# dkales/dpf-go

Measured on AMD Instinct MI355X. Metric: DPF leaf points/sec (EvalFull logN=20, batched keys) + AES blocks/sec, higher is better.
Workload: dtype u32

## Files before the change

### dpf-go_amd/csrc/dpf_capi.hip

```cpp
#include <hip/hip_runtime.h>
#include <sched.h>
#include <stdint.h>
#include <stdio.h>
#include <stdlib.h>
#include <string.h>
#include <sys/mman.h>

#include <algorithm>
#include <atomic>
#include <condition_variable>
#include <functional>
#include <memory>
#include <mutex>
#include <unordered_map>
#include <string>
#include <thread>
#include <vector>

#include "../../include/dpf_hip.h"
#include "dpf_internal.hpp"
#include "bs_kernels.hpp"
#include "dpf_kernels.hpp"
#include "pir_kernels.hpp"
#include "pir_update_plan.hpp"
// ... 313 lines not shown
    void* frontier;
};

TreeWs tree_ws(void* work, size_t nk, uint32_t stop) {
    uint8_t* p = static_cast<uint8_t*>(work);
    TreeWs w;
    w.ek = reinterpret_cast<uint32_t*>(p);
    p += align256(nk * dpfk::ek_words(stop) * 4);
    w.ekb = reinterpret_cast<uint32_t*>(p);
    p += align256(nk * dpfk::bs_key_words(stop) * 4);
    w.frontier = p;
    return w;
}

bool want_bs() { return g_aes_impl.load(std::memory_order_relaxed) == DPF_AES_BITSLICED; }

hipError_t expand_keys(const uint8_t* d_keys, size_t klen, size_t nk, uint32_t stop, const TreeWs& w, hipStream_t st,
                       bool bs) {
    if (bs) return dpfk::launch_unpack_both(d_keys, klen, nk, stop, w.ek, w.ekb, st);
    return dpfk::launch_unpack(d_keys, klen, nk, stop, w.ek, st);
}

hipError_t run_tree(const TreeWs& w, size_t k0, size_t n, uint32_t stop, uint32_t prefix_bits, uint64_t prefix,
                    uint8_t* out, uint64_t stride, hipStream_t st, bool bs) {
    if (bs && dpfk::bs_applicable(stop, prefix_bits))
        return dpfk::launch_evalfull_bs(w.ek + k0 * dpfk::ek_words(stop), w.ekb + k0 * dpfk::bs_key_words(stop), n, stop,
                                        prefix_bits, prefix, out, stride, w.frontier, st);
    return dpfk::launch_evalfull(w.ek + k0 * dpfk::ek_words(stop), n, stop, prefix_bits, prefix, out, stride, st);
}

hipError_t tree_from_keys(const uint8_t* d_keys, size_t klen, size_t nk, uint32_t stop, uint32_t prefix_bits,
                          uint64_t prefix, uint8_t* out, uint64_t stride, void* d_work, hipStream_t st, bool bs,
                          bool* expanded) {
    if (!bs && dpfk::evalfull_raw_ok(nk, stop, prefix_bits)) {
        *expanded = false;
        return dpfk::launch_evalfull_raw(d_keys, klen, nk, stop, prefix_bits, prefix, out, stride, st);
    }
    *expanded = true;
    const TreeWs w = tree_ws(d_work, nk, stop);
    hipError_t e = expand_keys(d_keys, klen, nk, stop, w, st, bs);
    return e != hipSuccess ? e : run_tree(w, 0, nk, stop, prefix_bits, prefix, out, stride, st, bs);
}

constexpr size_t kStageBytes = (size_t)32 << 20;
constexpr size_t kSlabMinOut = (size_t)8 << 20;

int ensure_staging(Dev& d, size_t chunk_cap) {
    if (!d.cst) {
        HIP_TRY(hipStreamCreateWithFlags(&d.cst, hipStreamNonBlocking));
        for (int i = 0; i < 2; ++i) {
            HIP_TRY(hipEventCreateWithFlags(&d.ev_k[i], hipEventDisableTiming));
            HIP_TRY(hipEventCreateWithFlags(&d.ev_c[i], hipEventDisableTiming));
        }
    }
    HIP_TRY(hipError_t(d.out.ensure(2 * chunk_cap)));
    for (int i = 0; i < 2; ++i) HIP_TRY(d.pin[i].ensure(chunk_cap));
    return DPF_OK;
}

bool prefault_output() {
    static const bool on = [] {
        const char* e = getenv("DPF_PREFAULT_OUTPUT");
        return e && e[0] == '1';
    }();
    return on;
}

void hint_hugepages(uint8_t* p, size_t n) {
    if (n < ((size_t)64 << 20) || !prefault_output()) return;
    const uintptr_t a = ((uintptr_t)p + ((1u << 21) - 1)) & ~(uintptr_t)((1u << 21) - 1);
    const uintptr_t e = ((uintptr_t)p + n) & ~(uintptr_t)((1u << 21) - 1);
    if (e > a) (void)madvise((void*)a, e - a, MADV_HUGEPAGE);
// ... 391 lines not shown
        if (!raw) HIP_TRY(expand_keys(dk, klen, 1, stop, w, d.st, bs));
        return pipeline_d2h(d, (size_t)1 << extra, sub, [&](size_t j, uint8_t* dbuf, size_t& bytes, size_t& off) {
            const uint64_t p = ((uint64_t)lo << extra) + j;
            if (raw) HIP_TRY(dpfk::launch_evalfull_raw(dk, klen, 1, stop, pb + extra, p, dbuf, sub, d.st));
            else HIP_TRY(run_tree(w, 0, 1, stop, pb + extra, p, dbuf, sub, d.st, bs));
            bytes = sub;
            off = lo * slab + j * sub;
            return DPF_OK;
        }, out + lo * slab, slab, lo * slab);
    });
}

int dpf_evalfull_subtree_dev(int device, const uint8_t* d_keys, size_t klen, size_t nkeys, uint32_t logN,
                             uint32_t prefix_bits, uint64_t prefix, uint8_t* d_out, void* d_work, void* stream) {
    if (int rc = check_key(klen, logN)) return rc;
    const uint32_t stop = stop_of(logN);
    if (prefix_bits > stop || (prefix_bits < 64 && (prefix >> prefix_bits) != 0))
        return fail(DPF_ERR_PARAM, "dpf: subtree prefix out of range");
    if (nkeys == 0) return DPF_OK;
    DeviceGuard g(device);
    CuScope cus(stream);
    const bool bs = want_bs();
    bool expanded = false;
    forget_expanded(d_work);
    HIP_TRY(tree_from_keys(d_keys, klen, nkeys, stop, prefix_bits, prefix, d_out, (uint64_t)16 << (stop - prefix_bits),
                           d_work, (hipStream_t)stream, bs, &expanded));
    if (expanded) note_expanded(d_work, nkeys, stop, bs);
    return DPF_OK;
}

int dpf_evalfull_batch_dev(int device, const uint8_t* d_keys, size_t klen, size_t nkeys, uint32_t logN,
                           uint8_t* d_out, void* d_work, void* stream) {
    return dpf_evalfull_subtree_dev(device, d_keys, klen, nkeys, logN, 0, 0, d_out, d_work, stream);
}

size_t dpf_eval_workspace_size(size_t nkeys, size_t pts_per_key, uint32_t logN) {
    return std::max<size_t>(16, eval_work_bytes(nkeys, pts_per_key, logN));
}

uint32_t dpf_eval_frontier_level(uint32_t logN, size_t pts_per_key) {
    return logN > 63 ? 0 : dpfk::eval_frontier_level(stop_of(logN), pts_per_key);
}

int dpf_eval_batch_dev(int device, const uint8_t* d_keys, size_t klen, size_t nkeys, const uint64_t* d_xs,
                       size_t ppk, uint32_t logN, uint8_t* d_out, void* d_work, size_t work_bytes, void* stream) {
    if (int rc = check_key(klen, logN, false)) return rc;
    if (nkeys == 0 || ppk == 0) return DPF_OK;
    const uint32_t stop = stop_of(logN);
    const size_t ekb = pir_ek_bytes(nkeys, logN);
    if (work_bytes < nkeys * dpfk::ek_words(stop) * 4) return fail(DPF_ERR_PARAM, "dpf: Eval workspace too small");
    if (d_xs == nullptr || d_out == nullptr || d_keys == nullptr || (reinterpret_cast<uintptr_t>(d_xs) & 7u) != 0)
        return fail(DPF_ERR_PARAM, "dpf: d_keys/d_xs/d_out must be device pointers, d_xs 8-byte aligned");
    DeviceGuard g(device);
    CuScope cus(stream);
    forget_expanded(d_work);
    HIP_TRY(dpfk::launch_unpack(d_keys, klen, nkeys, stop, (uint32_t*)d_work, (hipStream_t)stream));
    void* frontier = work_bytes > ekb ? (uint8_t*)d_work + ekb : nullptr;
    HIP_TRY(dpfk::launch_eval((const uint32_t*)d_work, stop, logN, d_xs, nkeys * ppk, ppk, d_out, frontier,
                              work_bytes > ekb ? work_bytes - ekb : 0, (hipStream_t)stream));
    return DPF_OK;
}

int dpf_expand_keys_dev(int device, const uint8_t* d_keys, size_t klen, size_t nkeys, uint32_t logN, void* d_work,
                        void* stream) {
    if (int rc = check_key(klen, logN)) return rc;
    DeviceGuard g(device);
// ... 486 lines not shown
```

### dpf-go_amd/csrc/dpf_kernels.hip

```cpp
#include <hip/hip_runtime.h>
#include <stdint.h>
#include <stdlib.h>

#include <algorithm>
#include <atomic>
#include <cmath>
#include <type_traits>
#include "aes_consts.hpp"
#include "aes_ttable.hpp"
#include "dpf_kernels.hpp"
#include "wave_prio.hpp"
#include "tree_ops.hpp"

namespace dpfk {

#ifdef DPF_WAVE_TIMES
constexpr uint64_t kWaveTimesMax = 1u << 16;
__device__ uint64_t g_wave_times[5 * kWaveTimesMax];
#endif

struct Ctx {
    const uint8_t* tab;
    uint32_t lo;
    KeySrc ks;
// ... 550 lines not shown
    const uint64_t pairs = nblocks / 2;
    if (pairs == 0) return hipSuccess;
    const dim3 grid((uint32_t)((pairs + kBlock - 1) / kBlock));
    if (right)
        hipLaunchKernelGGL(k_mmo_tt<true>, grid, dim3(kBlock), 0, st, reinterpret_cast<const uint4*>(in),
                           reinterpret_cast<uint4*>(out), pairs, reps);
    else
        hipLaunchKernelGGL(k_mmo_tt<false>, grid, dim3(kBlock), 0, st, reinterpret_cast<const uint4*>(in),
                           reinterpret_cast<uint4*>(out), pairs, reps);
    return hipGetLastError();
}

hipError_t launch_unpack(const uint8_t* keys, uint64_t key_len, uint64_t nkeys, uint32_t stop, uint32_t* ek,
                         hipStream_t st) {
    const uint64_t n = nkeys * ((uint64_t)stop + 2);
    if (n == 0) return hipSuccess;
    const uint32_t blocks = (uint32_t)((n + 255) / 256);
    hipLaunchKernelGGL(k_unpack, dim3(blocks), dim3(256), 0, st, keys, key_len, nkeys, stop, ek);
    return hipGetLastError();
}

static thread_local int t_cu_budget = 0;
void set_cu_budget(int cus) { t_cu_budget = cus; }
int cu_budget() { return t_cu_budget; }
int cu_count() {
    if (t_cu_budget > 0) return t_cu_budget;
    int dev = 0, cus = 256;
    if (hipGetDevice(&dev) != hipSuccess ||
        hipDeviceGetAttribute(&cus, hipDeviceAttributeMultiprocessorCount, dev) != hipSuccess)
        cus = 256;
    return cus;
}

static uint32_t pick_block(uint64_t n, uint32_t maxb) {
    const uint64_t cus = (uint64_t)cu_count();
    uint32_t b = 64;
    while (b < maxb && n > cus * b) b <<= 1;
    return b;
}

struct TreeShape {
    uint32_t d, block;
};
static TreeShape pick_shape(uint32_t span, uint64_t nkeys, bool nodes, uint32_t prefix_bits) {
    static const int forced = [] {
        const char* e = getenv("DPF_SUBTREE_DEPTH");
        return e ? atoi(e) : -1;
    }();
    const uint32_t dmax = span < kMaxD ? span : kMaxD;
    auto threads = [&](uint32_t dd) { return span - dd >= 40 ? ~0ull : nkeys << (span - dd); };
    auto block = [&](uint32_t dd) {
        return pick_block(threads(dd), !nodes && dd >= kBigMinD ? (uint32_t)kTreeBlockBig : (uint32_t)kTreeBlock);
    };
    if (forced >= 0) {
        const uint32_t d = dmax < (uint32_t)forced ? dmax : (uint32_t)forced;
        return {d, block(d)};
    }
    constexpr double kLat = 1.9e-6;
    constexpr double kPerWave = 0.2e-6;
    const double wave_slots = 64.0 * cu_count();
    uint32_t best = dmax;
    double best_t = 1e30;
    for (int dd = (int)dmax; dd >= 0; --dd) {
        const uint32_t d = (uint32_t)dd;
        double walk = (double)(span - d), lat = 0.0;
        const double w = (double)threads(d) / wave_slots;
        const double rounds = w > 16.0 ? std::ceil(w / 16.0) : 1.0;
        const double per = w > 16.0 ? 16.0 * kPerWave : std::max(kLat, w * kPerWave);
        const uint32_t W = 31u - (uint32_t)__builtin_clz(block(d));
        if (W >= 7 && span - d >= W) {
            walk = (double)(W - 6);
            lat = (double)(span + prefix_bits - d - W + 6) * kLat;
        }
        const double work = walk + (nodes ? 2.0 : 3.0) * (double)(1u << d) - 2.0;
        const double t = rounds * (lat + work * std::max(kLat, per));
        if (t < best_t * 0.98) {
            best_t = t;
            best = d;
        }
    }
    return {best, block(best)};
}

struct TreeLaunch {
    uint32_t d;
    uint32_t ltop;
    uint32_t units_log;
    uint64_t nunits, sub_base;
    dim3 grid, block;
};
static TreeLaunch tree_launch(uint64_t nkeys, uint32_t depth, uint32_t prefix_bits, uint64_t prefix, bool nodes) {
    const TreeShape sh = pick_shape(depth - prefix_bits, nkeys, nodes, prefix_bits);
    TreeLaunch t;
    t.d = sh.d;
    t.ltop = depth - sh.d;
    t.units_log = t.ltop - prefix_bits;
    t.nunits = nkeys << t.units_log;
    t.sub_base = prefix << t.units_log;
    t.grid = dim3((uint32_t)((t.nunits + sh.block - 1) / sh.block));
    t.block = dim3(sh.block);
    return t;
}
template <class F>
static void with_depth(uint32_t d, F&& f) {
    switch (d) {
        case 0: return f(std::integral_constant<int, 0>{});
        case 1: return f(std::integral_constant<int, 1>{});
        case 2: return f(std::integral_constant<int, 2>{});
        case 3: return f(std::integral_constant<int, 3>{});
        case 4: return f(std::integral_constant<int, 4>{});
        case 5: return f(std::integral_constant<int, 5>{});
        case 6: return f(std::integral_constant<int, 6>{});
        default: return f(std::integral_constant<int, 7>{});
    }
}

template <bool NODES>
static hipError_t launch_tree(const uint32_t* ek, uint64_t nkeys, uint32_t stop, uint32_t depth,
                              uint32_t prefix_bits, uint64_t prefix, uint8_t* out, uint8_t* out_t,
                              uint64_t out_stride, hipStream_t st) {
    const TreeLaunch t = tree_launch(nkeys, depth, prefix_bits, prefix, NODES);
    if (t.nunits == 0) return hipSuccess;
    with_depth(t.d, [&](auto dd) {
        constexpr int D = decltype(dd)::value;
        if (t.units_log >= 6)
            hipLaunchKernelGGL((k_evalfull<D, true, NODES>), t.grid, t.block, 0, st, ek, stop, t.nunits, t.units_log,
                               t.ltop, t.sub_base, out, out_t, out_stride);
        else
            hipLaunchKernelGGL((k_evalfull<D, false, NODES>), t.grid, t.block, 0, st, ek, stop, t.nunits, t.units_log,
                               t.ltop, t.sub_base, out, out_t, out_stride);
    });
    return hipGetLastError();
}

bool evalfull_raw_ok(uint64_t nkeys, uint32_t stop, uint32_t prefix_bits) {
    static const bool on = [] {
        const char* e = getenv("DPF_RAW_KEYS");
        return !(e && e[0] == '0');
    }();
    if (!on || nkeys == 0 || prefix_bits > stop) return false;
    return tree_launch(nkeys, stop, prefix_bits, 0, false).units_log >= 6;
}

hipError_t launch_evalfull_raw(const uint8_t* keys, uint64_t klen, uint64_t nkeys, uint32_t stop, uint32_t prefix_bits,
                               uint64_t prefix, uint8_t* out, uint64_t out_stride, hipStream_t st) {
    const TreeLaunch t = tree_launch(nkeys, stop, prefix_bits, prefix, false);
    if (t.units_log < 6) return hipErrorInvalidValue;
    const uint64_t kboff = (uintptr_t)keys & 3;
    const uint32_t* kw = reinterpret_cast<const uint32_t*>(keys - kboff);
    with_depth(t.d, [&](auto dd) {
        hipLaunchKernelGGL((k_evalfull<decltype(dd)::value, true, false, true>), t.grid, t.block, 0, st, kw, stop,
                           t.nunits, t.units_log, t.ltop, t.sub_base, out, nullptr, out_stride, klen, kboff);
    });
    return hipGetLastError();
}

hipError_t launch_nodes(const uint32_t* ek, uint64_t nkeys, uint32_t stop, uint32_t depth, uint32_t prefix_bits,
                        uint64_t prefix, uint8_t* seeds, uint8_t* ts, uint64_t stride, hipStream_t st) {
    return launch_tree<true>(ek, nkeys, stop, depth, prefix_bits, prefix, seeds, ts, stride, st);
}

hipError_t launch_evalfull(const uint32_t* ek, uint64_t nkeys, uint32_t stop, uint32_t prefix_bits,
                           uint64_t prefix, uint8_t* out, uint64_t out_stride, hipStream_t st) {
    return launch_tree<false>(ek, nkeys, stop, stop, prefix_bits, prefix, out, nullptr, out_stride, st);
}

uint32_t eval_frontier_level(uint32_t stop, uint64_t pts_per_key) {
    uint32_t L = 0;
    while (L < kMaxFrontierHbm && L < stop && (2ull << (L + 1)) <= pts_per_key) ++L;
    static const int shift = [] {
        const char* e = getenv("DPF_EVAL_LEVEL_SHIFT");
        return e && *e ? atoi(e) : 0;
    }();
    if (L >= 4 && shift > 0 && L + (uint32_t)shift < stop && L + (uint32_t)shift <= kMaxFrontierHbm) L += shift;
    return L >= 4 ? L : 0;
}

uint64_t eval_frontier_bytes(uint64_t nkeys, uint32_t stop, uint64_t pts_per_key) {
    const uint32_t L = eval_frontier_level(stop, pts_per_key);
    if (L == 0) return 0;
    return ((nkeys << L) * 16 + (nkeys << L) + 255) & ~255ull;
}

static std::atomic<int> g_eval_trie{[] {
    const char* e = getenv("DPF_EVAL_TRIE");
    return eval_trie_built() && e && e[0] == '1' ? 1 : 0;
}()};
// ... 8 lines not shown
    static const bool plain = [] {
        const char* e = getenv("DPF_EVAL_MODE");
        return e && e[0] == 'p';
    }();
    const uint64_t nkeys = nq / pts_per_key;
    uint32_t L = eval_frontier_level(stop, pts_per_key);
    if (logN > 63 || plain || frontier == nullptr || frontier_bytes < eval_frontier_bytes(nkeys, stop, pts_per_key)) L = 0;
    const uint4* fseed = nullptr;
    const uint8_t* ft = nullptr;
    if (L > 0) {
        uint8_t* fs = static_cast<uint8_t*>(frontier);
        uint8_t* fts = fs + (nkeys << L) * 16;
        hipError_t e = launch_tree<true>(ek, nkeys, stop, L, 0, 0, fs, fts, 1ull << L, st);
        if (e != hipSuccess) return e;
        fseed = reinterpret_cast<const uint4*>(fs);
        ft = fts;
    }
    if (L > 0 && trie_on() && nq == nkeys * pts_per_key && eval_trie_ok(stop, logN, pts_per_key, L))
        return launch_eval_trie(ek, stop, logN, xs, nkeys, pts_per_key, fseed, ft, L, out, st);
    static const int persist = [] {
        const char* e = getenv("DPF_EVAL_PERSIST");
        return e && *e ? atoi(e) : 1;
    }();
    const bool xs16 = (reinterpret_cast<uintptr_t>(xs) & 15u) == 0;
    if (persist && xs16 && L > 0 && pts_per_key % 128 == 0 && nq == nkeys * pts_per_key &&
        nq >= 2 * (uint64_t)kEvalPBlock) {
        const uint64_t want = (nq / 2 + kEvalPBlock - 1) / kEvalPBlock;
        const uint64_t cus = (uint64_t)cu_count();
        hipLaunchKernelGGL(k_eval_persist, dim3((uint32_t)(want < cus ? want : cus)), dim3(kEvalPBlock), 0, st, ek, stop,
                           logN, xs, nq, pts_per_key, fseed, ft, L, out);
        return hipGetLastError();
    }
    const uint64_t nthreads = (nq + 1) / 2;
    const uint32_t block = pick_block(nthreads, kBlock);
    const uint64_t blocks = (nthreads + block - 1) / block;
    if (blocks > 0x7fffffffull) return hipErrorInvalidValue;
    static const bool uni_on = [] {
        const char* e = getenv("DPF_EVAL_UNIFORM");
        return !(e && e[0] == '0');
    }();
    if (uni_on && pts_per_key % 128 == 0 && block % 64 == 0)
        hipLaunchKernelGGL(k_eval2<true>, dim3((uint32_t)blocks), dim3(block), 0, st, ek, stop, logN, xs, nq,
                           pts_per_key, fseed, ft, L, out);
    else
        hipLaunchKernelGGL(k_eval2<false>, dim3((uint32_t)blocks), dim3(block), 0, st, ek, stop, logN, xs, nq,
                           pts_per_key, fseed, ft, L, out);
    return hipGetLastError();
}

}
```

### dpf-go_amd/csrc/dpf_kernels.hpp

```cpp
#pragma once
#include <hip/hip_runtime.h>
#include <stdint.h>

namespace dpfk {

constexpr int kBlock = 512;
constexpr int kTreeBlock = 512;
constexpr int kTreeBlockBig = 1024;
constexpr int kTreeBlockMax = 1024;
constexpr uint32_t kBigMinD = 6;
constexpr uint32_t kFeedbackMinD = 6;
constexpr int kTreeWaves = 4;
constexpr uint32_t kMaxD = 7;
constexpr uint32_t kMaxFrontierHbm = 16;

void set_cu_budget(int cus);
int cu_budget();
int cu_count();

inline uint64_t ek_words(uint32_t stop) { return ((uint64_t)stop + 2) * 8; }

hipError_t launch_mmo_tt(const uint8_t* in, uint8_t* out, uint64_t nblocks, uint32_t right, uint32_t reps,
                         hipStream_t st);

hipError_t launch_unpack(const uint8_t* keys, uint64_t key_len, uint64_t nkeys, uint32_t stop, uint32_t* ek,
                         hipStream_t st);

hipError_t launch_evalfull(const uint32_t* ek, uint64_t nkeys, uint32_t stop, uint32_t prefix_bits,
                           uint64_t prefix, uint8_t* out, uint64_t out_stride, hipStream_t st);

bool evalfull_raw_ok(uint64_t nkeys, uint32_t stop, uint32_t prefix_bits);
hipError_t launch_evalfull_raw(const uint8_t* keys, uint64_t klen, uint64_t nkeys, uint32_t stop, uint32_t prefix_bits,
                               uint64_t prefix, uint8_t* out, uint64_t out_stride, hipStream_t st);

hipError_t launch_nodes(const uint32_t* ek, uint64_t nkeys, uint32_t stop, uint32_t depth, uint32_t prefix_bits,
                        uint64_t prefix, uint8_t* seeds, uint8_t* ts, uint64_t stride, hipStream_t st);

uint32_t eval_frontier_level(uint32_t stop, uint64_t pts_per_key);
int set_eval_trie(int on);
int get_eval_trie();
bool eval_trie_built();
bool eval_trie_ok(uint32_t stop, uint32_t logN, uint64_t pts_per_key, uint32_t L);
hipError_t launch_eval_trie(const uint32_t* ek, uint32_t stop, uint32_t logN, const uint64_t* xs, uint64_t nkeys,
                            uint64_t pts_per_key, const uint4* fseed, const uint8_t* ft, uint32_t L, uint8_t* out,
                            hipStream_t st);
uint64_t eval_frontier_bytes(uint64_t nkeys, uint32_t stop, uint64_t pts_per_key);
hipError_t launch_eval(const uint32_t* ek, uint32_t stop, uint32_t logN, const uint64_t* xs, uint64_t nq,
                       uint64_t pts_per_key, uint8_t* out, void* frontier, uint64_t frontier_bytes,
                       hipStream_t st);

}
```

### dpf-go_amd/dpf/__init__.py

```python
from __future__ import annotations

import ctypes
import os
from typing import Optional, Sequence, Tuple

import numpy as np

_HERE = os.path.dirname(os.path.abspath(__file__))
LIB_PATH = os.environ.get("DPF_LIB") or os.path.join(os.path.dirname(_HERE), "lib", "libdpf_hip.so")
HEADER_PATH = os.path.join(os.path.dirname(os.path.dirname(_HERE)), "include", "dpf_hip.h")

DPF_OK = 0
DPF_ERR_PARAM = -1
DPF_ERR_KEYLEN = -2
DPF_ERR_NODEV = -3
DPF_ERR_HIP = -4
DPF_ERR_NOMEM = -5
AES_TTABLE = 0
AES_BITSLICED = 1


class DPFPanic(RuntimeError):

    def __init__(self, code: int, msg: str):
# ... 43 lines not shown
    "dpf_get_aes_impl": (_int, []),
    "dpf_set_eval_kernel": (_int, [_int]),
    "dpf_get_eval_kernel": (_int, []),
    "dpf_set_pir_kernel": (_int, [_int]),
    "dpf_get_pir_kernel": (_int, []),
    "dpf_pir_kernel_for": (_int, [_sz, _u32, _u32]),
    "dpf_aes_mmo_dev": (_int, [_int, _int, _int, _vp, _vp, _sz, _u32, _vp]),
    "dpf_xor_fold_workspace_size": (_sz, []),
    "dpf_xor_fold_dev": (_int, [_int, _vp, _sz, _sz, _vp, _u64, _sz, _vp, _vp, _vp]),
    "dpf_pir_workspace_size": (_sz, [_sz, _u32, _u32]),
    "dpf_pir_answer_dev": (_int, [_int, _vp, _sz, _sz, _u32, _u32, _u64, _vp, _u64, _vp, _vp, _vp]),
    "dpf_pir_db_sliced_size": (_sz, [_u64]),
    "dpf_pir_db_slice_dev": (_int, [_int, _vp, _u64, _vp, _vp]),
    "dpf_pir_answer_sliced_dev": (_int, [_int, _vp, _sz, _sz, _u32, _u32, _u64, _vp, _u64, _vp, _vp, _vp]),
    "dpf_xor_fold_sliced_dev": (_int, [_int, _vp, _sz, _sz, _vp, _u64, _vp, _vp, _vp]),
    "dpf_set_fold_limits": (_int, [_u32, _u32]),
    "dpf_pir_db_sliced_size_wide": (_sz, [_u64, _sz]),
    "dpf_pir_db_slice_wide_dev": (_int, [_int, _vp, _u64, _sz, _vp, _vp]),
    "dpf_xor_fold_sliced_wide_dev": (_int, [_int, _vp, _sz, _sz, _vp, _u64, _sz, _vp, _vp, _vp]),
    "dpf_pir_answer_sliced_wide_dev": (_int, [_int, _vp, _sz, _sz, _u32, _u32, _u64, _vp, _u64, _sz, _vp, _vp, _vp]),
    "dpf_pir_answer_wide_dev": (_int, [_int, _vp, _sz, _sz, _u32, _u32, _u64, _vp, _u64, _sz, _vp, _vp, _vp]),
    "dpf_pir_db_update_sliced_wide_dev": (_int, [_int, _vp, _u64, _sz, _vp, _vp, _sz, _vp]),
    "dpf_pir_db_gather_sliced_wide_dev": (_int, [_int, _vp, _u64, _sz, _vp, _sz, _vp, _vp]),
    "dpf_pir_db_create_wide": (_int, [_u8p, _u64, _sz, _u32, _int, ctypes.POINTER(_vp)]),
    "dpf_pir_db_rec_bytes": (_sz, [_vp]),
    "dpf_pir_db_nrec": (_u64, [_vp]),
    "dpf_pir_db_update": (_int, [_vp, _u64p, _u8p, _sz]),
    "dpf_pir_db_read": (_int, [_vp, _u64p, _sz, _u8p]),
    "dpf_pir_db_create": (_int, [_u8p, _u64, _u32, _int, ctypes.POINTER(_vp)]),
    "dpf_pir_answer": (_int, [_vp, _u8p, _sz, _sz, _u8p]),
    "dpf_pir_db_free": (None, [_vp]),
    "dpf_stream_create_cu_masked": (_int, [_int, _u32, _u32, ctypes.POINTER(_vp)]),
    "dpf_stream_destroy": (_int, [_vp]),
}

_lib: Optional[ctypes.CDLL] = None


def lib() -> ctypes.CDLL:
    global _lib
    if _lib is None:
        if not os.path.exists(LIB_PATH):
            raise ImportError(f"{LIB_PATH} missing: build it with `make -C dpf-go_amd` (no CPU fallback exists)")
        try:
            import torch
        except ImportError:
            pass
        L = ctypes.CDLL(LIB_PATH)
        for name, (res, args) in SIGNATURES.items():
            f = getattr(L, name)
            f.restype = res
            f.argtypes = args
        _lib = L
    return _lib


def _check(rc: int) -> None:
    if rc != DPF_OK:
        msg = lib().dpf_last_error().decode(errors="replace")
        raise DPFPanic(rc, msg)


def _buf(a: np.ndarray):
    return a.ctypes.data_as(_u8p)


# ... 266 lines not shown
    if isinstance(mode, str):
        mode = {"auto": SMALL_AUTO, "gpu": SMALL_GPU, "host": SMALL_HOST}[mode]
    rc = lib().dpf_set_small_call_path(mode)
    if rc < 0:
        _check(rc)
    return rc


def get_small_call_path() -> int:
    return int(lib().dpf_get_small_call_path())


def small_call_max_logN() -> int:
    return int(lib().dpf_small_call_max_logN())


def aes_mmo_dev(d_in, d_out, nblocks: int, impl: int = AES_TTABLE, right: bool = False, reps: int = 1,
                device: int = 0, stream=None) -> None:
    _check(lib().dpf_aes_mmo_dev(device, impl, 1 if right else 0, _ptr(d_in), _ptr(d_out), nblocks, reps,
                                 _stream_handle(stream)))


def stream_create_cu_masked(cu_first: int, cu_count: int, device: int = 0):
    import torch
    h = _vp()
    _check(lib().dpf_stream_create_cu_masked(device, cu_first, cu_count, ctypes.byref(h)))
    return torch.cuda.ExternalStream(h.value, device=torch.device("cuda", device))


def stream_destroy(stream) -> None:
    _check(lib().dpf_stream_destroy(_stream_handle(stream)))


def xor_fold_workspace_size() -> int:
    return int(lib().dpf_xor_fold_workspace_size())


def xor_fold_dev(d_bits, bits_stride: int, nkeys: int, d_payload, nrec: int, rec_bytes: int, d_ans, d_work,
                 device: int = 0, stream=None) -> None:
    _check(lib().dpf_xor_fold_dev(device, _ptr(d_bits), bits_stride, nkeys, _ptr(d_payload), nrec, rec_bytes,
                                  _ptr(d_ans), _ptr(d_work), _stream_handle(stream)))


def pir_workspace_size(nkeys: int, logN: int, prefix_bits: int = 0) -> int:
    return int(lib().dpf_pir_workspace_size(nkeys, logN, prefix_bits))


def pir_answer_dev(d_keys, key_len_: int, nkeys: int, logN: int, d_db, nrec: int, d_ans, d_work,
                   prefix_bits: int = 0, prefix: int = 0, device: int = 0, stream=None) -> None:
    _check(lib().dpf_pir_answer_dev(device, _ptr(d_keys), key_len_, nkeys, logN, prefix_bits, prefix, _ptr(d_db),
                                    nrec, _ptr(d_ans), _ptr(d_work), _stream_handle(stream)))


def pir_db_sliced_size(nrec: int) -> int:
    return int(lib().dpf_pir_db_sliced_size(nrec))


def pir_db_slice_dev(d_db, nrec: int, d_dbs, device: int = 0, stream=None) -> None:
    _check(lib().dpf_pir_db_slice_dev(device, _ptr(d_db), nrec, _ptr(d_dbs), _stream_handle(stream)))


def pir_answer_sliced_dev(d_keys, key_len_: int, nkeys: int, logN: int, d_dbs, nrec: int, d_ans, d_work,
                          prefix_bits: int = 0, prefix: int = 0, device: int = 0, stream=None) -> None:
    _check(lib().dpf_pir_answer_sliced_dev(device, _ptr(d_keys), key_len_, nkeys, logN, prefix_bits, prefix,
                                           _ptr(d_dbs), nrec, _ptr(d_ans), _ptr(d_work), _stream_handle(stream)))

# ... 101 lines not shown
```

### include/dpf_hip.h

```cpp
#ifndef DPF_HIP_H
#define DPF_HIP_H

#include <stddef.h>
#include <stdint.h>

#ifdef __cplusplus
extern "C" {
#endif

#define DPF_OK 0
#define DPF_ERR_PARAM (-1)
#define DPF_ERR_KEYLEN (-2)
#define DPF_ERR_NODEV (-3)
#define DPF_ERR_HIP (-4)
#define DPF_ERR_NOMEM (-5)

const char* dpf_last_error(void);

size_t dpf_key_len(uint32_t logN);
size_t dpf_evalfull_len(uint32_t logN);
size_t dpf_workspace_size(size_t nkeys, uint32_t logN);

int dpf_gpu_init(int ngpus);
int dpf_gpu_init_devices(const int* ordinals, int n);
void dpf_gpu_shutdown(void);
int dpf_gpu_count(void);

int dpf_gen_seeded(uint64_t alpha, uint32_t logN, const uint8_t s0[16], const uint8_t s1[16], uint8_t* ka,
                   uint8_t* kb);
int dpf_gen(uint64_t alpha, uint32_t logN, uint8_t* ka, uint8_t* kb);
int dpf_gen_batch_seeded(const uint64_t* alphas, uint32_t logN, const uint8_t* s0s, const uint8_t* s1s, size_t n,
                         uint8_t* kas, uint8_t* kbs, int nthreads);

int dpf_keys_pack(const uint8_t* const* keys, const size_t* lens, size_t n, size_t key_len, uint8_t* out);
int dpf_keys_unpack(const uint8_t* packed, size_t key_len, size_t n, uint8_t* const* keys);

int dpf_eval(const uint8_t* key, size_t key_len, uint64_t x, uint32_t logN, uint8_t* out_bit);
int dpf_evalfull(const uint8_t* key, size_t key_len, uint32_t logN, uint8_t* out);
int dpf_evalfull_batch(const uint8_t* keys, size_t key_len, size_t nkeys, uint32_t logN, uint8_t* out, int ngpus);
int dpf_eval_batch(const uint8_t* keys, size_t key_len, size_t nkeys, const uint64_t* xs, size_t pts_per_key,
                   uint32_t logN, uint8_t* out, int ngpus);
int dpf_evalfull_split(const uint8_t* key, size_t key_len, uint32_t logN, uint8_t* out, int ngpus);

int dpf_evalfull_batch_dev(int device, const uint8_t* d_keys, size_t key_len, size_t nkeys, uint32_t logN,
                           uint8_t* d_out, void* d_work, void* stream);
int dpf_evalfull_subtree_dev(int device, const uint8_t* d_keys, size_t key_len, size_t nkeys, uint32_t logN,
                             uint32_t prefix_bits, uint64_t prefix, uint8_t* d_out, void* d_work, void* stream);
size_t dpf_eval_workspace_size(size_t nkeys, size_t pts_per_key, uint32_t logN);
uint32_t dpf_eval_frontier_level(uint32_t logN, size_t pts_per_key);
int dpf_eval_batch_dev(int device, const uint8_t* d_keys, size_t key_len, size_t nkeys, const uint64_t* d_xs,
                       size_t pts_per_key, uint32_t logN, uint8_t* d_out, void* d_work, size_t work_bytes,
                       void* stream);

int dpf_stream_create_cu_masked(int device, uint32_t cu_first, uint32_t cu_count, void** stream);
int dpf_stream_destroy(void* stream);

#define DPF_AES_TTABLE 0
#define DPF_AES_BITSLICED 1
int dpf_set_aes_impl(int impl);
int dpf_get_aes_impl(void);
#define DPF_EVAL_WALK 0
#define DPF_EVAL_TRIE 1
int dpf_set_eval_kernel(int kernel);
int dpf_get_eval_kernel(void);
#define DPF_SMALL_AUTO 0
#define DPF_SMALL_GPU 1
#define DPF_SMALL_HOST 2
int dpf_set_small_call_path(int mode);
int dpf_get_small_call_path(void);
uint32_t dpf_small_call_max_logN(void);
int dpf_aes_mmo_dev(int device, int impl, int right, const uint8_t* d_in, uint8_t* d_out, size_t nblocks,
                    uint32_t reps, void* stream);

int dpf_expand_keys_dev(int device, const uint8_t* d_keys, size_t key_len, size_t nkeys, uint32_t logN, void* d_work,
                        void* stream);
int dpf_evalfull_expanded_dev(int device, void* d_work, size_t nkeys, uint32_t logN, uint32_t prefix_bits,
                              uint64_t prefix, uint8_t* d_out, void* stream);
int dpf_forget_workspace(const void* d_work);


size_t dpf_pir_workspace_size(size_t nkeys, uint32_t logN, uint32_t prefix_bits);
int dpf_pir_answer_dev(int device, const uint8_t* d_keys, size_t key_len, size_t nkeys, uint32_t logN,
                       uint32_t prefix_bits, uint64_t prefix, const uint8_t* d_db, uint64_t nrec, uint8_t* d_ans,
                       void* d_work, void* stream);

size_t dpf_xor_fold_workspace_size(void);
int dpf_xor_fold_dev(int device, const uint8_t* d_bits, size_t bits_stride, size_t nkeys, const uint8_t* d_payload,
                     uint64_t nrec, size_t rec_bytes, uint8_t* d_ans, void* d_work, void* stream);
// ... 49 lines not shown
```

Measured before the change: 4704 billion.

## Split ragged key batches into per-depth tree segments with a cost-model planner

Replaces the single-shape subtree depth/block picker with a recursive planner that can split a key batch into segments. Full-round key counts run at a deeper subtree depth and the remainder runs at a shallower one, using a refined per-CU occupancy cost model. EvalFull now launches per segment, using raw-key kernels where a segment is uniform and unpack plus tree kernels otherwise. The aim is to cut tail-wave waste on ragged batch sizes, at the cost of extra kernel launches. It also exposes the plan through a C API and Python helper, and adds profiling scripts.

New measurement: 4713 billion (median of 4 runs). Within noise of the previous version (+0.2%).

```diff
diff --git a/dpf-go_amd/csrc/dpf_capi.hip b/dpf-go_amd/csrc/dpf_capi.hip
--- a/dpf-go_amd/csrc/dpf_capi.hip
+++ b/dpf-go_amd/csrc/dpf_capi.hip
@@ -369,12 +369,10 @@
 hipError_t tree_from_keys(const uint8_t* d_keys, size_t klen, size_t nk, uint32_t stop, uint32_t prefix_bits,
                           uint64_t prefix, uint8_t* out, uint64_t stride, void* d_work, hipStream_t st, bool bs,
                           bool* expanded) {
-    if (!bs && dpfk::evalfull_raw_ok(nk, stop, prefix_bits)) {
-        *expanded = false;
-        return dpfk::launch_evalfull_raw(d_keys, klen, nk, stop, prefix_bits, prefix, out, stride, st);
-    }
+    const TreeWs w = tree_ws(d_work, nk, stop);
+    if (!bs)
+        return dpfk::launch_evalfull_keys(d_keys, klen, nk, stop, prefix_bits, prefix, out, stride, w.ek, st, expanded);
     *expanded = true;
-    const TreeWs w = tree_ws(d_work, nk, stop);
     hipError_t e = expand_keys(d_keys, klen, nk, stop, w, st, bs);
     return e != hipSuccess ? e : run_tree(w, 0, nk, stop, prefix_bits, prefix, out, stride, st, bs);
 }
@@ -832,6 +830,19 @@
 int dpf_evalfull_batch_dev(int device, const uint8_t* d_keys, size_t klen, size_t nkeys, uint32_t logN,
                            uint8_t* d_out, void* d_work, void* stream) {
     return dpf_evalfull_subtree_dev(device, d_keys, klen, nkeys, logN, 0, 0, d_out, d_work, stream);
+}
+
+int dpf_tree_plan(size_t nkeys, uint32_t logN, uint32_t prefix_bits, uint32_t cus, uint64_t* segs, size_t cap) {
+    if (logN > 63) return fail(DPF_ERR_PARAM, "dpf: logN > 63");
+    const uint32_t stop = stop_of(logN);
+    if (prefix_bits > stop) return fail(DPF_ERR_PARAM, "dpf: subtree prefix out of range");
+    if (cus == 0 || (cap > 0 && segs == nullptr)) return fail(DPF_ERR_PARAM, "dpf: cus must be > 0 and segs hold cap segments");
+    const dpfk::TreePlan plan = dpfk::plan_tree(nkeys, stop - prefix_bits, prefix_bits, false, cus);
+    for (uint32_t i = 0; i < plan.n && i < cap; ++i) {
+        const dpfk::TreeSeg& s = plan.seg[i];
+        segs[4 * i] = s.key0, segs[4 * i + 1] = s.nkeys, segs[4 * i + 2] = s.d, segs[4 * i + 3] = s.block;
+    }
+    return (int)plan.n;
 }
 
 size_t dpf_eval_workspace_size(size_t nkeys, size_t pts_per_key, uint32_t logN) {
diff --git a/dpf-go_amd/csrc/dpf_kernels.hip b/dpf-go_amd/csrc/dpf_kernels.hip
--- a/dpf-go_amd/csrc/dpf_kernels.hip
+++ b/dpf-go_amd/csrc/dpf_kernels.hip
@@ -606,54 +606,12 @@
     return cus;
 }
 
-static uint32_t pick_block(uint64_t n, uint32_t maxb) {
-    const uint64_t cus = (uint64_t)cu_count();
-    uint32_t b = 64;
-    while (b < maxb && n > cus * b) b <<= 1;
-    return b;
-}
-
-struct TreeShape {
-    uint32_t d, block;
-};
-static TreeShape pick_shape(uint32_t span, uint64_t nkeys, bool nodes, uint32_t prefix_bits) {
+static TreePlan tree_plan(uint64_t nkeys, uint32_t depth, uint32_t prefix_bits, bool nodes) {
     static const int forced = [] {
         const char* e = getenv("DPF_SUBTREE_DEPTH");
         return e ? atoi(e) : -1;
     }();
-    const uint32_t dmax = span < kMaxD ? span : kMaxD;
-    auto threads = [&](uint32_t dd) { return span - dd >= 40 ? ~0ull : nkeys << (span - dd); };
-    auto block = [&](uint32_t dd) {
-        return pick_block(threads(dd), !nodes && dd >= kBigMinD ? (uint32_t)kTreeBlockBig : (uint32_t)kTreeBlock);
-    };
-    if (forced >= 0) {
-        const uint32_t d = dmax < (uint32_t)forced ? dmax : (uint32_t)forced;
-        return {d, block(d)};
-    }
-    constexpr double kLat = 1.9e-6;
-    constexpr double kPerWave = 0.2e-6;
-    const double wave_slots = 64.0 * cu_count();
-    uint32_t best = dmax;
-    double best_t = 1e30;
-    for (int dd = (int)dmax; dd >= 0; --dd) {
-        const uint32_t d = (uint32_t)dd;
-        double walk = (double)(span - d), lat = 0.0;
-        const double w = (double)threads(d) / wave_slots;
-        const double rounds = w > 16.0 ? std::ceil(w / 16.0) : 1.0;
-        const double per = w > 16.0 ? 16.0 * kPerWave : std::max(kLat, w * kPerWave);
-        const uint32_t W = 31u - (uint32_t)__builtin_clz(block(d));
-        if (W >= 7 && span - d >= W) {
-            walk = (double)(W - 6);
-            lat = (double)(span + prefix_bits - d - W + 6) * kLat;
-        }
-        const double work = walk + (nodes ? 2.0 : 3.0) * (double)(1u << d) - 2.0;
-        const double t = rounds * (lat + work * std::max(kLat, per));
-        if (t < best_t * 0.98) {
-            best_t = t;
-            best = d;
-        }
-    }
-    return {best, block(best)};
+    return plan_tree(nkeys, depth - prefix_bits, prefix_bits, nodes, (uint64_t)cu_count(), forced);
 }
 
 struct TreeLaunch {
@@ -663,17 +621,19 @@
     uint64_t nunits, sub_base;
     dim3 grid, block;
 };
-static TreeLaunch tree_launch(uint64_t nkeys, uint32_t depth, uint32_t prefix_bits, uint64_t prefix, bool nodes) {
-    const TreeShape sh = pick_shape(depth - prefix_bits, nkeys, nodes, prefix_bits);
+static TreeLaunch tree_launch(const TreeSeg& sg, uint32_t depth, uint32_t prefix_bits, uint64_t prefix) {
     TreeLaunch t;
-    t.d = sh.d;
-    t.ltop = depth - sh.d;
+    t.d = sg.d;
+    t.ltop = depth - sg.d;
     t.units_log = t.ltop - prefix_bits;
-    t.nunits = nkeys << t.units_log;
+    t.nunits = sg.nkeys << t.units_log;
     t.sub_base = prefix << t.units_log;
-    t.grid = dim3((uint32_t)((t.nunits + sh.block - 1) / sh.block));
-    t.block = dim3(sh.block);
+    t.grid = dim3((uint32_t)((t.nunits + sg.block - 1) / sg.block));
+    t.block = dim3(sg.block);
     return t;
+}
+static bool seg_uniform(const TreeSeg& sg, uint32_t depth, uint32_t prefix_bits) {
+    return depth - sg.d - prefix_bits >= 6;
 }
 template <class F>
 static void with_depth(uint32_t d, F&& f) {
@@ -690,11 +650,13 @@
 }
 
 template <bool NODES>
-static hipError_t launch_tree(const uint32_t* ek, uint64_t nkeys, uint32_t stop, uint32_t depth,
-                              uint32_t prefix_bits, uint64_t prefix, uint8_t* out, uint8_t* out_t,
-                              uint64_t out_stride, hipStream_t st) {
-    const TreeLaunch t = tree_launch(nkeys, depth, prefix_bits, prefix, NODES);
+static hipError_t launch_seg(const TreeSeg& sg, const uint32_t* ek, uint32_t stop, uint32_t depth, uint32_t prefix_bits,
+                             uint64_t prefix, uint8_t* out, uint8_t* out_t, uint64_t out_stride, hipStream_t st) {
+    const TreeLaunch t = tree_launch(sg, depth, prefix_bits, prefix);
     if (t.nunits == 0) return hipSuccess;
+    ek += sg.key0 * ek_words(stop);
+    out += sg.key0 * out_stride * (NODES ? sizeof(uint4) : 1);
+    if (out_t) out_t += sg.key0 * out_stride;
     with_depth(t.d, [&](auto dd) {
         constexpr int D = decltype(dd)::value;
         if (t.units_log >= 6)
@@ -707,26 +669,80 @@
     return hipGetLastError();
 }
 
-bool evalfull_raw_ok(uint64_t nkeys, uint32_t stop, uint32_t prefix_bits) {
+template <bool NODES>
+static hipError_t launch_tree(const uint32_t* ek, uint64_t nkeys, uint32_t stop, uint32_t depth,
+                              uint32_t prefix_bits, uint64_t prefix, uint8_t* out, uint8_t* out_t,
+                              uint64_t out_stride, hipStream_t st) {
+    const TreePlan plan = tree_plan(nkeys, depth, prefix_bits, NODES);
+    for (uint32_t i = 0; i < plan.n; ++i) {
+        const hipError_t e = launch_seg<NODES>(plan.seg[i], ek, stop, depth, prefix_bits, prefix, out, out_t, out_stride, st);
+        if (e != hipSuccess) return e;
+    }
+    return hipSuccess;
+}
+
+static bool raw_keys_on() {
     static const bool on = [] {
         const char* e = getenv("DPF_RAW_KEYS");
         return !(e && e[0] == '0');
     }();
-    if (!on || nkeys == 0 || prefix_bits > stop) return false;
-    return tree_launch(nkeys, stop, prefix_bits, 0, false).units_log >= 6;
+    return on;
+}
+
+bool evalfull_raw_ok(uint64_t nkeys, uint32_t stop, uint32_t prefix_bits) {
+    if (!raw_keys_on() || nkeys == 0 || prefix_bits > stop) return false;
+    const TreePlan plan = tree_plan(nkeys, stop, prefix_bits, false);
+    for (uint32_t i = 0; i < plan.n; ++i)
+        if (!seg_uniform(plan.seg[i], stop, prefix_bits)) return false;
+    return true;
+}
+
+static hipError_t launch_seg_raw(const TreeSeg& sg, const uint8_t* keys, uint64_t klen, uint32_t stop,
+                                 uint32_t prefix_bits, uint64_t prefix, uint8_t* out, uint64_t out_stride,
+                                 hipStream_t st) {
+    const TreeLaunch t = tree_launch(sg, stop, prefix_bits, prefix);
+    const uint8_t* k0 = keys + sg.key0 * klen;
+    const uint64_t kboff = (uintptr_t)k0 & 3;
+    const uint32_t* kw = reinterpret_cast<const uint32_t*>(k0 - kboff);
+    with_depth(t.d, [&](auto dd) {
+        hipLaunchKernelGGL((k_evalfull<decltype(dd)::value, true, false, true>), t.grid, t.block, 0, st, kw, stop,
+                           t.nunits, t.units_log, t.ltop, t.sub_base, out + sg.key0 * out_stride, nullptr, out_stride,
+                           klen, kboff);
+    });
+    return hipGetLastError();
 }
 
 hipError_t launch_evalfull_raw(const uint8_t* keys, uint64_t klen, uint64_t nkeys, uint32_t stop, uint32_t prefix_bits,
                                uint64_t prefix, uint8_t* out, uint64_t out_stride, hipStream_t st) {
-    const TreeLaunch t = tree_launch(nkeys, stop, prefix_bits, prefix, false);
-    if (t.units_log < 6) return hipErrorInvalidValue;
-    const uint64_t kboff = (uintptr_t)keys & 3;
-    const uint32_t* kw = reinterpret_cast<const uint32_t*>(keys - kboff);
-    with_depth(t.d, [&](auto dd) {
-        hipLaunchKernelGGL((k_evalfull<decltype(dd)::value, true, false, true>), t.grid, t.block, 0, st, kw, stop,
-                           t.nunits, t.units_log, t.ltop, t.sub_base, out, nullptr, out_stride, klen, kboff);
-    });
-    return hipGetLastError();
+    const TreePlan plan = tree_plan(nkeys, stop, prefix_bits, false);
+    for (uint32_t i = 0; i < plan.n; ++i)
+        if (!seg_uniform(plan.seg[i], stop, prefix_bits)) return hipErrorInvalidValue;
+    for (uint32_t i = 0; i < plan.n; ++i) {
+        const hipError_t e = launch_seg_raw(plan.seg[i], keys, klen, stop, prefix_bits, prefix, out, out_stride, st);
+        if (e != hipSuccess) return e;
+    }
+    return hipSuccess;
+}
+
+hipError_t launch_evalfull_keys(const uint8_t* keys, uint64_t klen, uint64_t nkeys, uint32_t stop, uint32_t prefix_bits,
+                                uint64_t prefix, uint8_t* out, uint64_t out_stride, uint32_t* ek, hipStream_t st,
+                                bool* expanded) {
+    const TreePlan plan = tree_plan(nkeys, stop, prefix_bits, false);
+    uint32_t unpacked = 0;
+    for (uint32_t i = 0; i < plan.n; ++i) {
+        const TreeSeg& sg = plan.seg[i];
+        hipError_t e;
+        if (raw_keys_on() && seg_uniform(sg, stop, prefix_bits)) {
+            e = launch_seg_raw(sg, keys, klen, stop, prefix_bits, prefix, out, out_stride, st);
+        } else {
+            ++unpacked;
+            e = launch_unpack(keys + sg.key0 * klen, klen, sg.nkeys, stop, ek + sg.key0 * ek_words(stop), st);
+            if (e == hipSuccess) e = launch_seg<false>(sg, ek, stop, stop, prefix_bits, prefix, out, nullptr, out_stride, st);
+        }
+        if (e != hipSuccess) return e;
+    }
+    *expanded = plan.n > 0 && unpacked == plan.n;
+    return hipSuccess;
 }
 
 hipError_t launch_nodes(const uint32_t* ek, uint64_t nkeys, uint32_t stop, uint32_t depth, uint32_t prefix_bits,
@@ -801,7 +817,7 @@
         return hipGetLastError();
     }
     const uint64_t nthreads = (nq + 1) / 2;
-    const uint32_t block = pick_block(nthreads, kBlock);
+    const uint32_t block = pick_block(nthreads, kBlock, (uint64_t)cu_count());
     const uint64_t blocks = (nthreads + block - 1) / block;
     if (blocks > 0x7fffffffull) return hipErrorInvalidValue;
     static const bool uni_on = [] {
diff --git a/dpf-go_amd/csrc/dpf_kernels.hpp b/dpf-go_amd/csrc/dpf_kernels.hpp
--- a/dpf-go_amd/csrc/dpf_kernels.hpp
+++ b/dpf-go_amd/csrc/dpf_kernels.hpp
@@ -2,16 +2,12 @@
 #include <hip/hip_runtime.h>
 #include <stdint.h>
 
+#include "tree_plan.hpp"
+
 namespace dpfk {
 
 constexpr int kBlock = 512;
-constexpr int kTreeBlock = 512;
-constexpr int kTreeBlockBig = 1024;
-constexpr int kTreeBlockMax = 1024;
-constexpr uint32_t kBigMinD = 6;
 constexpr uint32_t kFeedbackMinD = 6;
-constexpr int kTreeWaves = 4;
-constexpr uint32_t kMaxD = 7;
 constexpr uint32_t kMaxFrontierHbm = 16;
 
 void set_cu_budget(int cus);
@@ -32,6 +28,9 @@
 bool evalfull_raw_ok(uint64_t nkeys, uint32_t stop, uint32_t prefix_bits);
 hipError_t launch_evalfull_raw(const uint8_t* keys, uint64_t klen, uint64_t nkeys, uint32_t stop, uint32_t prefix_bits,
                                uint64_t prefix, uint8_t* out, uint64_t out_stride, hipStream_t st);
+hipError_t launch_evalfull_keys(const uint8_t* keys, uint64_t klen, uint64_t nkeys, uint32_t stop, uint32_t prefix_bits,
+                                uint64_t prefix, uint8_t* out, uint64_t out_stride, uint32_t* ek, hipStream_t st,
+                                bool* expanded);
 
 hipError_t launch_nodes(const uint32_t* ek, uint64_t nkeys, uint32_t stop, uint32_t depth, uint32_t prefix_bits,
                         uint64_t prefix, uint8_t* seeds, uint8_t* ts, uint64_t stride, hipStream_t st);
diff --git a/dpf-go_amd/csrc/tree_plan.hpp b/dpf-go_amd/csrc/tree_plan.hpp
--- /dev/null
+++ b/dpf-go_amd/csrc/tree_plan.hpp
@@ -0,0 +1,115 @@
+#pragma once
+#include <stdint.h>
+
+#include <algorithm>
+
+namespace dpfk {
+
+constexpr int kTreeBlock = 512;
+constexpr int kTreeBlockBig = 1024;
+constexpr int kTreeBlockMax = 1024;
+constexpr uint32_t kBigMinD = 6;
+constexpr int kTreeWaves = 4;
+constexpr uint32_t kMaxD = 7;
+constexpr uint32_t kCuWaves = 4 * kTreeWaves;
+
+inline uint32_t pick_block(uint64_t n, uint32_t maxb, uint64_t cus) {
+    uint32_t b = 64;
+    while (b < maxb && n > cus * b) b <<= 1;
+    return b;
+}
+
+inline uint64_t tree_threads(uint64_t nkeys, uint32_t span, uint32_t d) {
+    return span - d >= 40 || (nkeys << (span - d)) >> (span - d) != nkeys ? ~0ull : nkeys << (span - d);
+}
+
+inline uint32_t tree_block(uint64_t nkeys, uint32_t span, uint32_t d, bool nodes, uint64_t cus) {
+    const uint64_t n = tree_threads(nkeys, span, d);
+    const bool big = !nodes && d >= kBigMinD && n >= cus * (uint64_t)kTreeBlockBig;
+    return pick_block(n, big ? (uint32_t)kTreeBlockBig : (uint32_t)kTreeBlock, cus);
+}
+
+inline uint64_t tree_round_keys(uint32_t span, uint32_t d, uint64_t cus) {
+    const uint64_t slots = (uint64_t)kCuWaves * 64 * cus;
+    if (span - d >= 40) return 0;
+    const uint64_t k = slots >> (span - d);
+    return (k << (span - d)) == slots ? k : 0;
+}
+
+constexpr double kLat = 1.9e-6;
+constexpr double kPerWave = 0.2e-6;
+constexpr double kLaunchGap = 2.0e-6;
+inline double tree_launch_time(uint64_t nkeys, uint32_t span, uint32_t d, uint32_t prefix_bits, bool nodes,
+                               uint64_t cus) {
+    const uint64_t n = tree_threads(nkeys, span, d);
+    const uint32_t b = tree_block(nkeys, span, d, nodes, cus);
+    const uint64_t groups = n / b + (n % b != 0);
+    const uint64_t on_cu = (groups + cus - 1) / cus;
+    const uint64_t hold = b > (uint32_t)kTreeBlock ? 1 : 2;
+    const double rounds = (double)((on_cu + hold - 1) / hold);
+    const double w = (double)(std::min(on_cu, hold) * (b / 64));
+    const double per = std::max(kLat, (rounds > 1.0 ? (double)kCuWaves : w) * kPerWave);
+    double walk = (double)(span - d), lat = 0.0;
+    const uint32_t W = 31u - (uint32_t)__builtin_clz(b);
+    if (W >= 7 && span - d >= W) {
+        walk = (double)(W - 6);
+        lat = (double)(span + prefix_bits - d - W + 6) * kLat;
+    }
+    const double work = walk + (nodes ? 2.0 : 3.0) * (double)(1u << d) - 2.0;
+    return rounds * (lat + work * per);
+}
+
+struct TreeSeg {
+    uint64_t key0, nkeys;
+    uint32_t d, block;
+};
+struct TreePlan {
+    uint32_t n = 0;
+    TreeSeg seg[kMaxD + 1];
+    double t = 0.0;
+};
+
+inline TreePlan plan_tree_below(uint64_t key0, uint64_t nkeys, uint32_t span, uint32_t prefix_bits, bool nodes,
+                                uint64_t cus, uint32_t dmax) {
+    TreePlan best;
+    best.t = 1e30;
+    for (int dd = (int)dmax; dd >= 0; --dd) {
+        const uint32_t d = (uint32_t)dd;
+        const double one = tree_launch_time(nkeys, span, d, prefix_bits, nodes, cus);
+        if (one < best.t * 0.98) {
+            best.n = 1;
+            best.seg[0] = {key0, nkeys, d, tree_block(nkeys, span, d, nodes, cus)};
+            best.t = one;
+        }
+        const uint64_t kd = tree_round_keys(span, d, cus);
+        if (d == 0 || kd == 0 || nkeys <= kd || nkeys % kd == 0) continue;
+        const uint64_t full = nkeys / kd * kd;
+        const TreePlan rest = plan_tree_below(key0 + full, nkeys - full, span, prefix_bits, nodes, cus, d - 1);
+        const double t = tree_launch_time(full, span, d, prefix_bits, nodes, cus) + kLaunchGap + rest.t;
+        if (t < best.t * 0.98) {
+            best.n = 1 + rest.n;
+            best.seg[0] = {key0, full, d, tree_block(full, span, d, nodes, cus)};
+            std::copy(rest.seg, rest.seg + rest.n, best.seg + 1);
+            best.t = t;
+        }
+    }
+    return best;
+}
+
+inline TreePlan plan_tree(uint64_t nkeys, uint32_t span, uint32_t prefix_bits, bool nodes, uint64_t cus,
+                          int forced_d = -1) {
+    const uint32_t dmax = span < kMaxD ? span : kMaxD;
+    if (cus == 0) cus = 1;
+    if (nkeys == 0) return TreePlan{};
+    if (forced_d >= 0) {
+        const uint32_t d = dmax < (uint32_t)forced_d ? dmax : (uint32_t)forced_d;
+        TreePlan p;
+        p.n = 1;
+        p.seg[0] = {0, nkeys, d, tree_block(nkeys, span, d, nodes, cus)};
+        p.t = tree_launch_time(nkeys, span, d, prefix_bits, nodes, cus);
+        return p;
+    }
+    return plan_tree_below(0, nkeys, span, prefix_bits, nodes, cus, dmax);
+}
+
+}
diff --git a/dpf-go_amd/dpf/__init__.py b/dpf-go_amd/dpf/__init__.py
--- a/dpf-go_amd/dpf/__init__.py
+++ b/dpf-go_amd/dpf/__init__.py
@@ -99,6 +99,7 @@
     "dpf_pir_db_free": (None, [_vp]),
     "dpf_stream_create_cu_masked": (_int, [_int, _u32, _u32, ctypes.POINTER(_vp)]),
     "dpf_stream_destroy": (_int, [_vp]),
+    "dpf_tree_plan": (_int, [_sz, _u32, _u32, _u32, _u64p, _sz]),
 }
 
 _lib: Optional[ctypes.CDLL] = None
@@ -431,6 +432,15 @@
     _check(lib().dpf_stream_destroy(_stream_handle(stream)))
 
 
+def tree_plan(nkeys: int, logN: int, prefix_bits: int = 0, cus: int = 256) -> list:
+    cap = 8
+    segs = (ctypes.c_uint64 * (4 * cap))()
+    n = lib().dpf_tree_plan(nkeys, logN, prefix_bits, cus, segs, cap)
+    if n < 0:
+        _check(n)
+    return [tuple(int(v) for v in segs[4 * i:4 * i + 4]) for i in range(n)]
+
+
 def xor_fold_workspace_size() -> int:
     return int(lib().dpf_xor_fold_workspace_size())
 
diff --git a/include/dpf_hip.h b/include/dpf_hip.h
--- a/include/dpf_hip.h
+++ b/include/dpf_hip.h
@@ -54,6 +54,8 @@
 
 int dpf_stream_create_cu_masked(int device, uint32_t cu_first, uint32_t cu_count, void** stream);
 int dpf_stream_destroy(void* stream);
+
+int dpf_tree_plan(size_t nkeys, uint32_t logN, uint32_t prefix_bits, uint32_t cus, uint64_t* segs, size_t cap);
 
 #define DPF_AES_TTABLE 0
 #define DPF_AES_BITSLICED 1
diff --git a/profiles/ragged_batch/cmp_dumps.py b/profiles/ragged_batch/cmp_dumps.py
--- /dev/null
+++ b/profiles/ragged_batch/cmp_dumps.py
@@ -0,0 +1,12 @@
+import os
+import sys
+
+import numpy as np
+
+a, b, n = sys.argv[1], sys.argv[2], sys.argv[3]
+fa, fb = sorted(os.listdir(a)), sorted(os.listdir(b))
+assert fa == fb and fa, (fa, fb)
+for f in fa:
+    x, y = np.load(os.path.join(a, f)), np.load(os.path.join(b, f))
+    assert x.shape == y.shape and np.array_equal(x, y), f"nkeys={n}: {f} differs"
+print(f"nkeys={n}: {', '.join(fa)} equal ({sum(np.load(os.path.join(a, f)).size for f in fa)} values)")
diff --git a/profiles/ragged_batch/probe_shape.py b/profiles/ragged_batch/probe_shape.py
--- /dev/null
+++ b/profiles/ragged_batch/probe_shape.py
@@ -0,0 +1,48 @@
+import json
+import os
+import sys
+import time
+
+ROOT = os.path.dirname(os.path.dirname(os.path.dirname(os.path.abspath(__file__))))
+sys.path[:0] = [os.path.join(ROOT, "dpf-go_amd"), os.path.join(ROOT, "oracle")]
+import numpy as np
+import torch
+import dpf
+from dpf import synth
+
+nk, logN, cus = int(sys.argv[1]), int(sys.argv[2]), int(sys.argv[3])
+iters = int(sys.argv[4]) if len(sys.argv) > 4 else 300
+assert dpf.gpu_init(1) >= 1
+dev = torch.device("cuda", 0)
+al, s0, s1 = synth.key_seeds(nk, logN, first=99)
+ka, _ = dpf.gen_batch_seeded(al, logN, s0, s1)
+kl, ol = dpf.key_len(logN), dpf.evalfull_len(logN)
+d_keys = torch.from_numpy(ka.reshape(-1)).to(dev)
+d_work = torch.empty(dpf.workspace_size(nk, logN), dtype=torch.uint8, device=dev)
+out = torch.zeros(nk * ol, dtype=torch.uint8, device=dev)
+S = dpf.stream_create_cu_masked(0, cus) if cus else torch.cuda.current_stream(dev)
+
+
+def run(n):
+    for _ in range(n):
+        dpf.evalfull_batch_dev(d_keys, kl, nk, logN, out, d_work, stream=S)
+
+
+t0 = time.perf_counter()
+while time.perf_counter() - t0 < 0.5:
+    run(20)
+    S.synchronize()
+reps = []
+for _ in range(5):
+    S.synchronize()
+    t0 = time.perf_counter()
+    run(iters)
+    S.synchronize()
+    reps.append((time.perf_counter() - t0) / iters * 1e6)
+plan = dpf.tree_plan(nk, logN, 0, cus or 256) if hasattr(dpf, "tree_plan") else None
+print(json.dumps({"nkeys": nk, "logN": logN, "cus": cus, "forced_d": os.environ.get("DPF_SUBTREE_DEPTH"),
+                  "us_per_call_median": round(float(np.median(reps)), 2), "us_min": round(min(reps), 2),
+                  "us_max": round(max(reps), 2), "plan": plan}), flush=True)
+if cus:
+    torch.cuda.synchronize()
+    dpf.stream_destroy(S)
diff --git a/profiles/ragged_batch/summarize.py b/profiles/ragged_batch/summarize.py
--- /dev/null
+++ b/profiles/ragged_batch/summarize.py
@@ -0,0 +1,16 @@
+import glob
+import json
+import os
+import sys
+
+import numpy as np
+
+d = sys.argv[1]
+rows = {}
+for path in sorted(glob.glob(os.path.join(d, "*_*.jsonl"))):
+    which, n = os.path.basename(path)[:-6].split("_")
+    ms = [json.loads(ln)["ms_per_step"] for ln in open(path) if ln.strip().startswith("{")]
+    rows[(int(n), which)] = ms
+for (n, which), ms in sorted(rows.items()):
+    print(f"{n:6d} {which:7s} runs={len(ms)} median={np.median(ms):.4f} min={min(ms):.4f} max={max(ms):.4f} "
+          f"spread={max(ms) - min(ms):.4f}")
```
